# possoj/Spacecraft-Pose-Estimation-Framework

Measured on AMD Instinct MI355X. Metric: images/sec at 512×512 batch 64, 1/2/4/8 MI355X; pose err vs fp32 ref, higher is better.
Workload: dtype fp16mx; 1 GPU; C3: full net + decode, 512x512, batch 64 per GPU, fp16mx schedule; global_batch=64, image_size=512, parallelism=frame-parallel x1 (RCCL weight bcast), inflight_batches=3, frame_buffers=6

## Files before the change

spacecraft-pose-estimation-framework_amd/csrc/api_core.cpp:

```cpp
#include <string.h>

#include <algorithm>

#include "spef_ctx.hpp"

static thread_local std::string g_err;

int fail(int code, const std::string& msg) {
  g_err = msg;
  return code;
}
namespace spef {
int report_error(int code, const std::string& msg) { return fail(code, msg); }
}

int num_cus() {
  static int cus[32] = {};
  int dev = 0;
  if (hipGetDevice(&dev) != hipSuccess) dev = 0;
  dev &= 31;
  if (!cus[dev] && hipDeviceGetAttribute(&cus[dev], hipDeviceAttributeMultiprocessorCount, dev) != hipSuccess)
    cus[dev] = 256;
  return cus[dev];
}
// ... 35 lines not shown
  return SPEF_OK;
}

void free_workspace(spef_ctx* c) {
  for (void*& b : c->buf) {
    if (b) hipFree(b);
    b = nullptr;
  }
  if (c->pooled) hipFree(c->pooled);
  c->pooled = nullptr;
  if (c->kpfeat) hipFree(c->kpfeat);
  c->kpfeat = nullptr;
  if (c->kppart) hipFree(c->kppart);
  c->kppart = nullptr;
  c->ws_B = c->ws_H = c->ws_W = 0;
  c->buf_bytes = 0;
}

struct OptionDesc {
  int option;
  int spef_ctx::*field;
  bool flag;
  int lo, hi;
  const char* msg;
};
static const OptionDesc kOptions[] = {
    {SPEF_OPT_FUSE_BLOCKS, &spef_ctx::fuse, true, 0, 0, nullptr},
    {SPEF_OPT_IRB_VARIANT, &spef_ctx::irb_variant, false, 0, 0, nullptr},
    {SPEF_OPT_TEST_FAIL_BCAST, &spef_ctx::test_fail_bcast, false, 0, 3, "SPEF_OPT_TEST_FAIL_BCAST: 0..3"},
    {SPEF_OPT_PW_GEMM, &spef_ctx::gemm, true, 0, 0, nullptr},
    {SPEF_OPT_Q8_ROLESPLIT, &spef_ctx::q8_rolesplit, false, 0, 1, "SPEF_OPT_Q8_ROLESPLIT: 0 or 1"},
    {SPEF_OPT_MX_KERNELS, &spef_ctx::mx_kernels, true, 0, 0, nullptr},
    {SPEF_OPT_TRIM, &spef_ctx::trim, false, 0, 3, "SPEF_OPT_TRIM: bits 0-1"},
    {SPEF_OPT_WAVESPEC, &spef_ctx::wavespec, false, 0, 2, "SPEF_OPT_WAVESPEC: 0, 1 or 2"},
};

extern "C" {

int spef_abi_version(void) { return SPEF_ABI_VERSION; }

const char* spef_last_error(void) { return g_err.c_str(); }

int spef_init(int device, spef_ctx** out) {
  if (!out) return fail(SPEF_ERR_ARG, "out is null");
  int n = 0;
  HIP_TRY(hipGetDeviceCount(&n));
  if (device < 0 || device >= n) return fail(SPEF_ERR_ARG, "device index out of range");
  hipDeviceProp_t prop;
  HIP_TRY(hipGetDeviceProperties(&prop, device));
  if (strncmp(prop.gcnArchName, "gfx950", 6) != 0)
    return fail(SPEF_ERR_ARG, std::string("SPEF kernels are built for gfx950 only, device is ") + prop.gcnArchName);
  spef_ctx* c = new spef_ctx();
  c->device = device;
  *out = c;
  return SPEF_OK;
}

int spef_destroy(spef_ctx* c) {
  if (!c) return SPEF_OK;
  Dev d(c->device);
  free_workspace(c);
  if (c->d_data) hipFree(c->d_data);
  if (c->d_ori_bins) hipFree(c->d_ori_bins);
  if (c->d_pos_grid) hipFree(c->d_pos_grid);
  if (c->kp3d) hipFree(c->kp3d);
  if (c->kp_model) hipFree(c->kp_model);
// ... 119 lines not shown
```

spacecraft-pose-estimation-framework_amd/csrc/api_schedule.cpp:

```cpp
#include <math.h>

#include <initializer_list>

#include "spef_ctx.hpp"

namespace {

struct Act {
  void* p;
  int h, w, ch;
  bool f16;
};

inline void advance(Act& a, void* y, int h, int w, uint32_t ch, bool f16 = false) { a = Act{y, h, w, (int)ch, f16}; }

void* free_buf(const spef_ctx* c, std::initializer_list<const void*> busy) {
  for (void* b : c->buf) {
    bool used = false;
    for (const void* u : busy) used |= (u == b);
    if (!used) return b;
  }
  return nullptr;
}

// ... 139 lines not shown
int irb_step_x2(const Run& r, const OpDesc& op, const Block& g, Act& a) {
  spef_ctx* c = r.c;
  hipStream_t s = r.s;
  const int B = r.B, h = a.h, w = a.w, OH = g.OH, OW = g.OW;
  void* x = a.p;
  const bool cur16 = a.f16;
  void* y = free_buf(c, {x});
  const double hp = (op.hidden + 31) & ~31u;
  const bool o16 = r.out16(op);
  const int io = (cur16 ? 1 : 0) | (o16 ? 2 : 0);
  float* scratch = (float*)free_buf(c, {x, y});
  const X2Block blk{g.cin, g.hid, g.cout, g.stride, g.expand, g.res};
  const int cus = num_cus();
  const X2Plan plan = x2_irb_plan(blk, B, OH, OW, scratch != nullptr, io, cus);
  if (!plan.known) return fail(SPEF_ERR_ARG, "fp16x2 schedule: unsupported inverted-residual geometry");
  const double ib = cur16 ? 2 : 4, ob = o16 ? 2 : 4;
  const double bytes = (double)g.M * op.cin * ib + (double)g.M2 * op.cout * ob +
                       (g.expand ? hp * ((op.cin + 31) & ~31u) * 4 : 0) + hp * 48 +
                       ((op.cout + 15) & ~15u) * (hp * 4 + 4);
  char key[96];
  const bool mxk = r.mx && c->mx_kernels &&
                   mx_irb_supported(g.cin, g.hid, g.cout, g.stride, g.expand, g.res, cur16, o16);
  const bool mxlean = (c->trim & 2) != 0;
  const char* kn = mxk ? (mxlean && !mx_irb_lean_fits(g.cin, g.cout, o16, h, w, OH, OW) ? "mx_irb_kernel_wide"
                                                                                       : "mx_irb_kernel")
                       : plan.kernel_name();
  snprintf(key, sizeof(key), "%s<%u,%u,%u,s%u>", kn ? kn : "x2_irb_kernel", op.cin, op.hidden, op.cout, op.stride);
  const Wts wt = weights(c, op);
  HIP_TRY(prof_launch(c, s, key, bytes, irb_flops(op, g), [&] {
    if (mxk)
      return launch_mx_irb(g.cin, g.hid, g.cout, g.stride, g.res, cur16, o16, x, wt.w0, wt.b0, (const float*)wt.w1,
                           wt.b1, wt.w2, wt.b2, y, B, h, w, OH, OW, s, mxlean);
    return launch_x2_irb(blk, plan, {x, wt.w0, wt.b0, (const float*)wt.w1, wt.b1, wt.w2, wt.b2, y, B, h, w, OH, OW,
                                     scratch, io, cus}, s);
  }));
  advance(a, y, OH, OW, op.cout, o16);
  return SPEF_OK;
}

bool fused16_applies(const Run& r, const Block& g, const Act& a) {
  return !r.f32 && r.c->fuse && (int64_t)a.h * a.w >= r.c->fuse_min_hw &&
         irb_supported(g.cin, g.hid, g.cout, g.stride, g.expand, g.res);
}

int irb_step_fused16(const Run& r, const OpDesc& op, const Block& g, Act& a) {
  spef_ctx* c = r.c;
  hipStream_t s = r.s;
  const int B = r.B, h = a.h, w = a.w, dt = r.dt, OH = g.OH, OW = g.OW;
  void* x = a.p;
  void* y = free_buf(c, {x});
  const double bytes = (double)g.M * op.cin * 2 + (double)g.M2 * op.cout * 2 +
                       (g.expand ? pw_bytes(0, op.cin, op.hidden, false) : 0) + 40.0 * op.hidden +
                       pw_bytes(0, op.hidden, op.cout, false);
  const bool pipe3 = c->wavespec >= 2 && irp_supported(g.cin, g.hid, g.cout, g.stride, g.expand, g.res);
  const bool wspec = !pipe3 && c->wavespec && irw_supported(g.cin, g.hid, g.cout, g.stride, g.expand, g.res);
  char key[96];
  snprintf(key, sizeof(key), "%s<%u,%u,%u,s%u>", pipe3 ? "irp_kernel" : wspec ? "irw_kernel" : "irb_kernel",
           op.cin, op.hidden, op.cout, op.stride);
  const Wts wt = weights(c, op);
  HIP_TRY(prof_launch(c, s, key, bytes, irb_flops(op, g), [&] {
    if (pipe3)
      return launch_irp(c->irb_variant, dt, g.cin, g.hid, g.cout, g.stride, g.res, x, wt.w0, wt.b0, wt.w1, wt.b1, wt.w2,
                        wt.b2, y, B, h, w, OH, OW, s);
    if (wspec)
      return launch_irw(c->irb_variant, dt, g.cin, g.hid, g.cout, g.stride, g.res, x, wt.w0, wt.b0, wt.w1, wt.b1, wt.w2,
                        wt.b2, y, B, h, w, OH, OW, s);
    return launch_irb(c->irb_variant, dt, g.cin, g.hid, g.cout, g.stride, g.expand, g.res, x, wt.w0, wt.b0, wt.w1,
// ... 437 lines not shown
```

spacecraft-pose-estimation-framework_amd/csrc/k_x2_irw.hip:

```cpp
#include "spef_kernels.hpp"
#include "x2_common.hpp"

namespace spef {

#ifndef SPEF_X2_GLDS
#define SPEF_X2_GLDS 1
#endif
#ifndef SPEF_X2_GLDS_S2
#define SPEF_X2_GLDS_S2 1
#endif
template <int CIN, int HID, int COUT, int S, int TH, int TW, int WCO, bool PST, int P = 1>
struct X2wGeom {
  static constexpr int NE = 4, ND = 4, NW = NE + ND;
  static constexpr int IH = (TH - 1) * S + 3, IW = (TW - 1) * S + 3;
  static constexpr int PIN = IH * IW, PIN16 = (PIN + 15) / 16, PINP = PIN16 * 16;
  static constexpr int CINP = (CIN + 31) / 32 * 32, KS = CINP / 32;
  static constexpr int WES = CINP + 16;
  static constexpr int WPS = 48;
  using SL = X2Slab<S, PINP>;
  static constexpr int NCH = (HID + 31) / 32, HIDP = NCH * 32;
  static constexpr int NCL = NCH / P;
  static constexpr int NCT = (COUT + 15) / 16, NPC = NCT * 16;
  static constexpr int POUT16 = TH * TW / 16;
  static constexpr int WP = ND / WCO, QPW = POUT16 / WP, NCTW = NCT / WCO;
  static constexpr int EPT = (PIN16 + NE - 1) / NE;
  static constexpr int SLAB_B = SL::FLOATS * 4;
  static constexpr int SE_B = 2 * 32 * WES * 2 + 32 * 4;
  static constexpr int SD_B = (9 * 32 + 32) * 4;
  static constexpr int SP_B = PST ? 2 * NPC * WPS * 2 : 0;
  static constexpr bool GL = SPEF_X2_GLDS && COUT == 160 && (S == 1 || SPEF_X2_GLDS_S2);
  static constexpr int SE_BQ = (SE_B + 1023) / 1024 * 1024, SD_BQ = (SD_B + 1023) / 1024 * 1024;
  static constexpr int SP_BQ = (SP_B + 1023) / 1024 * 1024, DP_BQ = SD_BQ + SP_BQ;
  static constexpr int NIE = SE_BQ / 1024, NID = DP_BQ / 1024;
  static constexpr int IEW = (NIE + NE - 1) / NE, IDW = (NID + ND - 1) / ND;
  static constexpr int SE_STR = GL ? SE_BQ : SE_B, SD_STR = GL ? DP_BQ : SD_B, SP_STR = GL ? DP_BQ : SP_B;
  static constexpr int OFF_SE = 2 * SLAB_B;
  static constexpr int OFF_SD = GL ? OFF_SE + 2 * SE_BQ : OFF_SE + 2 * SE_B;
  static constexpr int OFF_SP = GL ? OFF_SD + SD_BQ : OFF_SD + 2 * SD_B;
  static constexpr int OFF_TR = GL ? OFF_SD + 2 * DP_BQ : OFF_SP + 2 * SP_B;
  static constexpr int OFF_ST = OFF_TR + 16 * 24 * 4;
  static constexpr int LDS_BYTES = OFF_ST + (SPEF_X2_STAMP ? 8 * 4 * 64 : 0);
  static constexpr int NPE = 2 * 32 * (CINP / 8) + 8, NPD = 9 * 8 + 8, NPP = PST ? 2 * NPC * 4 : 0;
  static constexpr int NPIECE = (NPE + NPD + NPP + NE * 64 - 1) / (NE * 64);
  static_assert(CIN % 8 == 0 && COUT % 4 == 0 && HID % 8 == 0, "channel counts");
  static_assert(TH * TW % 16 == 0 && POUT16 % WP == 0 && ND % WCO == 0 && NCT % WCO == 0, "tile split");
  static_assert(EPT <= 32 && NCH % P == 0 && NCL >= 2, "validity mask / hidden parts / pipeline depth");
  static_assert(SE_B % 16 == 0 && SD_B % 16 == 0 && SP_B % 16 == 0 && SLAB_B % 16 == 0, "16-B aligned stages");
  static_assert(LDS_BYTES <= 163840, "LDS budget");
};

#ifndef SPEF_X2_DWB
#define SPEF_X2_DWB 2
#endif
#ifndef SPEF_X2_ROWS
#define SPEF_X2_ROWS 1
#endif
#ifndef SPEF_X2_DWB2_CIN
#define SPEF_X2_DWB2_CIN 96
#endif
template <int CIN, int HID, int COUT, int S, int TH, int TW, bool RES, int WCO, bool PST, int P = 1, bool PT = false>
__global__ __launch_bounds__(8 * 64) __attribute__((amdgpu_waves_per_eu(2, 2))) void x2_irw_kernel(
    const float* __restrict__ X, const _Float16* __restrict__ We, const float* __restrict__ be,
    const float* __restrict__ Wd, const float* __restrict__ bd, const _Float16* __restrict__ Wp,
    const float* __restrict__ bp, float* __restrict__ Y, int H, int W, int OH, int OW, int tiles_x, int tiles_y,
    uint32_t nwg, size_t pstride, uint32_t ntile) {
  using G = X2wGeom<CIN, HID, COUT, S, TH, TW, WCO, PST, P>;
  using SL = typename G::SL;
  static_assert(!PT || (P == 1 && G::NCL % 2 == 0), "persistent tiles: one hidden part, even chunk count");
  extern __shared__ __attribute__((aligned(16))) char smem[];
  const int tid = threadIdx.x, wave = tid >> 6, lane = tid & 63;
  const int r16 = lane & 15, kg = lane >> 4;
  uint32_t L = xcd_remap(blockIdx.x, nwg);
  const bool stamp_wg = SPEF_X2_STAMP && L == 0;
  auto stamp = [&](int c, int slot) {
    if constexpr (SPEF_X2_STAMP) {
      if (stamp_wg && lane == 0 && c < 64)
        reinterpret_cast<uint32_t*>(smem + G::OFF_ST)[c * 8 + slot] = (uint32_t)__builtin_amdgcn_s_memtime();
    }
  };
  const uint32_t L0 = L;
  const int nt = PT ? (int)((ntile - L0 + nwg - 1) / nwg) : 1;
  const int GT = nt * G::NCL;
  const int part = (int)(L % (uint32_t)P);
  L /= (uint32_t)P;
  const int cb = part * G::NCL;
  auto tile_of = [&](uint32_t Lt, int& b_, int& oy0_, int& ox0_) {
    const int tx_ = (int)(Lt % (uint32_t)tiles_x);
    Lt /= (uint32_t)tiles_x;
    b_ = (int)(Lt / (uint32_t)tiles_y);
    oy0_ = (int)(Lt % (uint32_t)tiles_y) * TH;
    ox0_ = tx_ * TW;
  };
// ... 492 lines not shown
        if (c == G::NCL - SPEF_X2_RES_AHEAD || c == G::NCL - 1) {
          int b_, oy_, ox_;
          tile_of(L0 + (uint32_t)(g / G::NCL) * nwg, b_, oy_, ox_);
          if (c == G::NCL - SPEF_X2_RES_AHEAD) {
            fetch_res(b_, oy_, ox_);
          } else {
            float4 bn[G::NCTW];
#pragma unroll
            for (int t = 0; t < G::NCTW; ++t)
              bn[t] = *reinterpret_cast<const float4*>(bp + (wc * G::NCTW + t) * 16 + 4 * kg);
            epilogue(b_, oy_, ox_);
#pragma unroll
            for (int t = 0; t < G::NCTW; ++t)
#pragma unroll
              for (int q = 0; q < G::QPW; ++q) acc[q][t] = f32x4{bn[t].x, bn[t].y, bn[t].z, bn[t].w};
          }
        }
      }
      if (wr == 0) stamp(g, 6);
      __syncthreads();
    }
    if constexpr (!PT) epilogue(b, oy0, ox0);
    if (wr == 0) stamp(0, 7);
  }
  if constexpr (SPEF_X2_STAMP) {
    __syncthreads();
    if (stamp_wg && tid < 8 * 64) {
      const int n = 8 * (GT < 64 ? GT : 64);
      if (tid < n) reinterpret_cast<uint32_t*>(Y)[tid] = reinterpret_cast<const uint32_t*>(smem + G::OFF_ST)[tid];
    }
  }
}

template <int P, bool RES>
__global__ __launch_bounds__(256) void x2_split_reduce_kernel(const float* __restrict__ parts, size_t pstride,
                                                              const float* __restrict__ bias,
                                                              const float* __restrict__ X, float* __restrict__ Y,
                                                              size_t n4, int cout4) {
  const size_t i = (size_t)blockIdx.x * 256 + threadIdx.x;
  if (i >= n4) return;
  float4 v = reinterpret_cast<const float4*>(parts)[i];
#pragma unroll
  for (int p = 1; p < P; ++p) {
    const float4 u = reinterpret_cast<const float4*>(parts + p * pstride)[i];
    v.x += u.x; v.y += u.y; v.z += u.z; v.w += u.w;
  }
  const float4 bb = reinterpret_cast<const float4*>(bias)[i % (size_t)cout4];
  v.x += bb.x; v.y += bb.y; v.z += bb.z; v.w += bb.w;
  if constexpr (RES) {
    const float4 r = reinterpret_cast<const float4*>(X)[i];
    v.x += r.x; v.y += r.y; v.z += r.z; v.w += r.w;
  }
  reinterpret_cast<float4*>(Y)[i] = v;
}
template <int CIN, int HID, int COUT, int S, bool EXPAND, bool RES, int TH, int TW, int NW, int WCO, int KIND, int P>
static hipError_t x2_split_go(X2Row<CIN, HID, COUT, S, EXPAND, RES, TH, TW, NW, WCO, KIND, P>, const X2Args& a,
                              hipStream_t s) {
  static_assert(EXPAND && NW == 8, "role-split blocks expand, 4 + 4 waves");
  constexpr bool PT = KIND == 3 && P == 1;
  using G = X2wGeom<CIN, HID, COUT, S, TH, TW, WCO, KIND != 2, P>;
  TileGrid g;
  hipError_t e = tile_grid(g, a.OH, a.OW, TH, TW, a.B, P);
  if (e != hipSuccess) return e;
  auto k = x2_irw_kernel<CIN, HID, COUT, S, TH, TW, RES, WCO, KIND != 2, P, PT>;
  static DevOnce attr_set;
  if ((e = lds_attr_once(attr_set, k, G::LDS_BYTES)) != hipSuccess) return e;
  const size_t pstride = (size_t)a.B * a.OH * a.OW * COUT;
  if (P > 1 && !a.scratch) return hipErrorInvalidValue;
  const uint32_t grid = PT ? x2_persistent_grid(g.nwg, a.num_cu) : g.nwg;
  k<<<grid, G::NW * 64, G::LDS_BYTES, s>>>((const float*)a.x, (const _Float16*)a.we, a.be, a.wd, a.bd,
                                           (const _Float16*)a.wp, a.bp, P > 1 ? a.scratch : (float*)a.y, a.H, a.W,
                                           a.OH, a.OW, g.tiles_x, g.tiles_y, grid, pstride, g.nwg);
  if constexpr (P > 1) {
    const size_t n4 = pstride / 4;
    x2_split_reduce_kernel<P, RES><<<(unsigned)((n4 + 255) / 256), 256, 0, s>>>(a.scratch, pstride, a.bp,
                                                                                 (const float*)a.x, (float*)a.y, n4,
                                                                                 COUT / 4);
  }
  return hipGetLastError();
}

hipError_t launch_x2_split(const X2Block& b, const X2Plan& p, const X2Args& a, hipStream_t s) {
  return x2_visit_row<1, 3>(b, p, hipErrorNotSupported, [&](auto row) { return x2_split_go(row, a, s); });
}

}
```

spacecraft-pose-estimation-framework_amd/csrc/spef_ctx.hpp:

```cpp
#pragma once
#include "../../include/spef.h"

#include <hip/hip_runtime.h>

#include <array>
#include <string>
#include <vector>

#include "spef_blob.hpp"
#include "spef_kernels.hpp"
#include "spef_tuning.hpp"

using namespace spef;

#define SPEF_INTERNAL __attribute__((visibility("hidden")))

static const int kKpSplits = 60;

SPEF_INTERNAL int fail(int code, const std::string& msg);

#define HIP_TRY(expr)                                                                                  \
  do {                                                                                                 \
    hipError_t e_ = (expr);                                                                            \
    if (e_ != hipSuccess) return fail(SPEF_ERR_HIP, std::string(#expr) + ": " + hipGetErrorString(e_)); \
// ... 1 lines not shown

struct spef_ctx {
  int device = 0;
  BlobHeader hdr{};
  std::vector<OpDesc> ops;
  uint8_t* d_data = nullptr;
  size_t data_bytes = 0;
  bool loaded = false;
  int ws_B = 0, ws_H = 0, ws_W = 0;
  size_t buf_bytes = 0;
  void* buf[4] = {nullptr, nullptr, nullptr, nullptr};
  float* pooled = nullptr;
  float* kpfeat = nullptr;
  float* kppart = nullptr;
  float* kp3d = nullptr;
  double* kp_model = nullptr;
  int kp_n = 0;
  double camK[9] = {0};
  float cam_nu = 0.f, cam_nv = 0.f;
  EpnpDist kp_dist = {0, 0, 0, 0, 0, 0};
  double* d_ori_bins = nullptr;
  int n_ori_bins = 0;
  double* d_pos_grid = nullptr;
  int n_pos_bins = 0;
  int fuse = 1;
  int64_t fuse_min_hw = 0;
  int gemm = 1;
  int irb_variant = -1;
  int wavespec = 2;
  int q8_rolesplit = 0;
  int test_fail_bcast = 0;
  int mx_kernels = 1;
  int trim = 3;
  std::vector<double> q8_sw, q8_bias;
  std::vector<int32_t> q8_wsum;
  double q8_sl = 0.0;
  int32_t* q8_fc_init = nullptr;
  float* q8_fc_sc = nullptr;
  int q8_fc_hw = 0, q8_fc_tb = 0;
  float q8_s_img = 0.f;
  int q8_last_bits = 8, q8_pool_bits = 8, q8_fc_bias_bits = 8;
  int pre_key[4] = {0, 0, 0, 0};
  int* pre_bh = nullptr;
  int* pre_bv = nullptr;
  int pre_ksh = 0, pre_ksv = 0, pre_y0 = 0, pre_ht = 0;
  uint8_t* pre_tmp = nullptr;
  size_t pre_tmp_bytes = 0;
  std::vector<std::array<int64_t, 3>> q8_res;
  bool profiling = false;
  struct Rec {
    std::string key;
    hipEvent_t a, b;
    double bytes, flops;
  };
  std::vector<Rec> recs;
  std::vector<hipEvent_t> pool;
  size_t pool_next = 0;
};

struct spef_observer {
  int device = 0;
  int n_blocks = 0, n_taps = 0;
  std::vector<std::array<uint32_t, 7>> geom;
  uint64_t* state = nullptr;
  uint64_t* tap(int t) const { return state + (size_t)t * (OBS_COUNTERS + OBS_BINS); }
};
// ... 68 lines not shown
```

spacecraft-pose-estimation-framework_amd/csrc/spef_kernels.hpp:

```cpp
#pragma once
#include <hip/hip_runtime.h>
#include <stddef.h>
#include <stdint.h>

#include <string>

#include "x2_plan.hpp"

namespace spef {

int report_error(int code, const std::string& msg);

enum Dtype : int {
  DT_F16 = 1, DT_BF16 = 2, DT_I8 = 3, DT_F32 = 4,
  DT_X2 = 5,
  DT_MX = 6
};
enum Epi : int { EPI_NONE = 0, EPI_RELU = 1, EPI_RES = 2, EPI_RELU_F32 = 3  };
enum InLayout : int { IN_U8_NHWC = 0, IN_F32_NCHW = 1 };

hipError_t launch_stem(int dtype, int in_layout, const void* in, const float* w, const float* bias, void* y,
                       int B, int H, int W, int OH, int OW, hipStream_t s);

hipError_t launch_pw(int dtype, int epi, const void* x, const void* wt, const float* bias, const void* r,
// ... 20 lines not shown
int irb_dw_mode(int dtype, int hid, bool expand, int stride);
hipError_t launch_irb(int variant, int dtype, int cin, int hid, int cout, int stride, bool expand, bool res, const void* x,
                      const void* we, const float* be, const void* wd, const float* bd, const void* wp,
                      const float* bp, void* y, int B, int H, int W, int OH, int OW, hipStream_t s);

bool irp_supported(int cin, int hid, int cout, int stride, bool expand, bool res);
hipError_t launch_irp(int variant, int dtype, int cin, int hid, int cout, int stride, bool res, const void* x, const void* we,
                      const float* be, const void* wd, const float* bd, const void* wp, const float* bp, void* y, int B,
                      int H, int W, int OH, int OW, hipStream_t s);
bool irw_supported(int cin, int hid, int cout, int stride, bool expand, bool res);
hipError_t launch_irw(int variant, int dtype, int cin, int hid, int cout, int stride, bool res, const void* x, const void* we,
                      const float* be, const void* wd, const float* bd, const void* wp, const float* bp, void* y,
                      int B, int H, int W, int OH, int OW, hipStream_t s);

hipError_t launch_front(int dtype, const void* x, const void* wsp, const float* bs, const void* wd, const float* bd,
                        const void* wp, const float* bp, void* y, int B, int H, int W, int OH, int OW, hipStream_t s);

hipError_t launch_gemm_f32(int epi, const void* x, const void* wt, const float* bias, const void* r, void* y,
                           int64_t M, int K, int N, hipStream_t s);
const char* gemm_f32_key(int N);
bool x2_irb_supported(int cin, int hid, int cout, int stride, bool expand, bool res);
const char* x2_irb_kernel_name(int cin, int hid, int cout, int stride, bool expand, bool res, int B, int OH, int OW,
                               bool scratch, int io, int num_cu);
struct X2Args {
  const void* x;
  const void* we;
  const float *be, *wd, *bd;
  const void* wp;
  const float* bp;
  void* y;
  int B, H, W, OH, OW;
  float* scratch;
  int io, num_cu;
};
hipError_t launch_x2_irb(const X2Block& b, const X2Plan& p, const X2Args& a, hipStream_t s);
hipError_t launch_x2_slab(const X2Block& b, const X2Plan& p, const X2Args& a, hipStream_t s);
hipError_t launch_x2_split(const X2Block& b, const X2Plan& p, const X2Args& a, hipStream_t s);
hipError_t launch_x2_stage3(const X2Block& b, const X2Plan& p, const X2Args& a, hipStream_t s);
bool mx_irb_supported(int cin, int hid, int cout, int stride, bool expand, bool res, bool in16, bool out16);
hipError_t launch_mx_irb(int cin, int hid, int cout, int stride, bool res, bool in16, bool out16, const void* x,
                         const void* we,
                         const float* be, const float* wd, const float* bd, const void* wp, const float* bp, void* y,
                         int B, int H, int W, int OH, int OW, hipStream_t s, bool lean = true);
bool mx_irb_lean_fits(int cin, int cout, bool out16, int H, int W, int OH, int OW);
hipError_t launch_mx_front(const void* x, const void* wsp, const float* bs, const float* wd, const float* bd,
                           const void* wp, const float* bp, void* y, int B, int H, int W, int OH, int OW,
                           hipStream_t s);
hipError_t launch_x2_front(const void* x, const void* wsx, const float* bs, const float* wd, const float* bd,
                           const void* wp, const float* bp, void* y, int B, int H, int W, int OH, int OW, hipStream_t s,
                           bool out16 = false);
hipError_t launch_x2_pw_relu(const void* x, const void* wt, const float* bias, float* y, int64_t M, int K, int N,
                             hipStream_t s, bool wide = true);
bool x2_pw_pool_supported(int HW, int N);
hipError_t launch_x2_pw_pool(const void* x, const void* wt, const float* bias, float* part, float* pooled, int B,
                             int HW, int K, int N, hipStream_t s, bool wide = true);
hipError_t launch_mean_hw(const float* x, float* pooled, int B, int HW, int C, hipStream_t s);

hipError_t launch_fc_splitk(const float* x, const float* w, const float* bias, float* out, int n, int B, int K,
                            int splits, float* part, hipStream_t s);

struct EpnpDist {
  double k1, k2, p1, p2, k3;
  int on;
};
hipError_t launch_epnp(const float* raw, int B, int n, const float* kp3d, const double* model, const double* K,
                       float nu, float nv, const EpnpDist& dist, int apply_sigmoid, float* kp_out, float* quat,
// ... 132 lines not shown
```

spacecraft-pose-estimation-framework_amd/csrc/spef_tuning.hpp:

```cpp
#pragma once

enum spef_tuning_option {
  SPEF_OPT_FUSE_MIN_HW = 2,
  SPEF_OPT_PW_GEMM = 3,
  SPEF_OPT_IRB_VARIANT = 4,
  SPEF_OPT_TEST_FAIL_BCAST = 5,
  SPEF_OPT_MX_KERNELS = 8,
  SPEF_OPT_TRIM = 9
};
```

spacecraft-pose-estimation-framework_amd/spef_amd/_lib.py:

```python
from __future__ import annotations

import ctypes as C
import os

from . import _build

OK, ERR_ARG, ERR_HIP, ERR_BLOB, ERR_STATE, ERR_NUMERIC, ERR_COMM = range(7)
IN_U8_NHWC, IN_F32_NCHW = 0, 1
REGRESSION, CLASSIFICATION, KEYPOINTS = 0, 1, 2
ABI_VERSION = 4
COMM_ID_BYTES = 128
METRIC_IDS = {'l2': 0, 'kl': 1, 'js': 2, 'hellinger': 3, 'tv': 4, 'wasserstein': 5}
OPT_FUSE_BLOCKS, OPT_WAVESPEC, OPT_Q8_ROLESPLIT = 1, 6, 7
OPT_FUSE_MIN_HW, OPT_PW_GEMM, OPT_IRB_VARIANT, OPT_TEST_FAIL_BCAST = 2, 3, 4, 5
OPT_MX_KERNELS = 8
OPT_TRIM = 9
OPT_TRIM_DEFAULT = 3

_vp, _i, _sz = C.c_void_p, C.c_int, C.c_size_t
_ip = C.POINTER(C.c_int)
SIGNATURES = {
    'spef_abi_version': (_i, []),
    'spef_last_error': (C.c_char_p, []),
    'spef_init': (_i, [_i, C.POINTER(_vp)]),
    'spef_destroy': (_i, [_vp]),
    'spef_load_weights': (_i, [_vp, _vp, _sz]),
    'spef_load_weights_device': (_i, [_vp, _vp, _sz]),
    'spef_model_info': (_i, [_vp, _ip, _ip, _ip, _ip, _ip]),
    'spef_reserve': (_i, [_vp, _i, _i, _i]),
    'spef_preprocess': (_i, [_vp, _vp, _i, _i, _i, _vp, _i, _i, _vp]),
    'spef_forward': (_i, [_vp, _vp, _i, _i, _i, _i, _vp, _vp, _vp]),
    'spef_backbone': (_i, [_vp, _vp, _i, _i, _i, _i, _vp, _vp]),
    'spef_probe': (_i, [_vp, _vp, _i, _i, _i, _i, _i, _vp, _ip, _ip, _ip, _vp]),
    'spef_set_decode_tables': (_i, [_vp, _vp, _i, _vp, _i]),
    'spef_decode': (_i, [_vp, _i, _i, _vp, _i, _vp, _i, _i, _vp, _vp, _vp, _vp, _vp, _vp]),
    'spef_decode_cov': (_i, [_vp, _i, _i, _vp, _i, _vp, _i, _vp, _vp, _i, _vp, _vp, _vp, _vp, _vp]),
    'spef_video_create': (_i, [_vp, _i, _i, C.c_float, C.c_float, C.c_float, C.c_float, C.POINTER(_vp)]),
    'spef_video_reset': (_i, [_vp, _i, _vp]),
    'spef_video_set_state': (_i, [_vp, _i, _vp, _vp, _vp, _vp, _vp]),
    'spef_video_step': (_i, [_vp, _vp, _vp, _vp, _i, _i, _vp, _vp, _vp, _vp, _vp, _vp, _vp, _vp, _vp]),
    'spef_video_destroy': (_i, [_vp]),
    'spef_score_create': (_i, [_vp, _i, _i, _i, C.POINTER(_vp)]),
    'spef_score_reset': (_i, [_vp, _i, _vp]),
    'spef_score_step': (_i, [_vp, _i, _vp, _vp, _vp, _vp, _vp, _i, _i, _vp, _vp]),
    'spef_score_finalize': (_i, [_vp, _vp, _vp]),
    'spef_score_log': (_i, [_vp, _i, _i, _i, _i, _vp, _vp, _vp]),
    'spef_score_destroy': (_i, [_vp]),
    'spef_track_create': (_i, [_vp, _i, _vp, C.POINTER(_vp)]),
    'spef_track_reset': (_i, [_vp, _i, _vp]),
    'spef_track_get_state': (_i, [_vp, _i, _i, _vp, _vp]),
# ... 89 lines not shown
```

Baseline: 61390 images/sec.

## Add warp-specialized staged x2 IRB kernel with async global-to-LDS weight pipeline

```diff
diff --git a/spacecraft-pose-estimation-framework_amd/csrc/api_core.cpp b/spacecraft-pose-estimation-framework_amd/csrc/api_core.cpp
--- a/spacecraft-pose-estimation-framework_amd/csrc/api_core.cpp
+++ b/spacecraft-pose-estimation-framework_amd/csrc/api_core.cpp
@@ -91,6 +91,7 @@
     {SPEF_OPT_Q8_ROLESPLIT, &spef_ctx::q8_rolesplit, false, 0, 1, "SPEF_OPT_Q8_ROLESPLIT: 0 or 1"},
     {SPEF_OPT_MX_KERNELS, &spef_ctx::mx_kernels, true, 0, 0, nullptr},
     {SPEF_OPT_TRIM, &spef_ctx::trim, false, 0, 3, "SPEF_OPT_TRIM: bits 0-1"},
+    {SPEF_OPT_X2_STAGE, &spef_ctx::x2_stage, false, 0, 1, "SPEF_OPT_X2_STAGE: 0 or 1"},
     {SPEF_OPT_WAVESPEC, &spef_ctx::wavespec, false, 0, 2, "SPEF_OPT_WAVESPEC: 0, 1 or 2"},
 };
 
diff --git a/spacecraft-pose-estimation-framework_amd/csrc/api_schedule.cpp b/spacecraft-pose-estimation-framework_amd/csrc/api_schedule.cpp
--- a/spacecraft-pose-estimation-framework_amd/csrc/api_schedule.cpp
+++ b/spacecraft-pose-estimation-framework_amd/csrc/api_schedule.cpp
@@ -195,7 +195,7 @@
       return launch_mx_irb(g.cin, g.hid, g.cout, g.stride, g.res, cur16, o16, x, wt.w0, wt.b0, (const float*)wt.w1,
                            wt.b1, wt.w2, wt.b2, y, B, h, w, OH, OW, s, mxlean);
     return launch_x2_irb(blk, plan, {x, wt.w0, wt.b0, (const float*)wt.w1, wt.b1, wt.w2, wt.b2, y, B, h, w, OH, OW,
-                                     scratch, io, cus}, s);
+                                     scratch, io, cus, c->x2_stage}, s);
   }));
   advance(a, y, OH, OW, op.cout, o16);
   return SPEF_OK;
diff --git a/spacecraft-pose-estimation-framework_amd/csrc/k_x2_irw.hip b/spacecraft-pose-estimation-framework_amd/csrc/k_x2_irw.hip
--- a/spacecraft-pose-estimation-framework_amd/csrc/k_x2_irw.hip
+++ b/spacecraft-pose-estimation-framework_amd/csrc/k_x2_irw.hip
@@ -8,6 +8,9 @@
 #endif
 #ifndef SPEF_X2_GLDS_S2
 #define SPEF_X2_GLDS_S2 1
+#endif
+#ifndef SPEF_X2_DPE_WIDE
+#define SPEF_X2_DPE_WIDE 0
 #endif
 template <int CIN, int HID, int COUT, int S, int TH, int TW, int WCO, bool PST, int P = 1>
 struct X2wGeom {
@@ -47,7 +50,82 @@
   static_assert(EPT <= 32 && NCH % P == 0 && NCL >= 2, "validity mask / hidden parts / pipeline depth");
   static_assert(SE_B % 16 == 0 && SD_B % 16 == 0 && SP_B % 16 == 0 && SLAB_B % 16 == 0, "16-B aligned stages");
   static_assert(LDS_BYTES <= 163840, "LDS budget");
+  static constexpr int SLF = SL::FLOATS + 16 * 24;
+  static constexpr int DPE = COUT == 64 ? NID : SPEF_X2_DPE_WIDE < NID ? SPEF_X2_DPE_WIDE : NID;
+  static constexpr int ST_LDS = 2 * SLF * 4 + 2 * SE_BQ + 2 * DP_BQ + (SPEF_X2_STAMP ? 8 * 4 * 64 : 0);
 };
+
+template <class G>
+__device__ __forceinline__ const char* x2w_stage_src(bool estage, int off, const _Float16* We, const float* be,
+                                                     const float* Wd, const float* bd, const _Float16* Wp) {
+  if (estage) {
+    constexpr int EW_B = 2 * 32 * G::WES * 2, ROW_B = G::WES * 2;
+    if (off < EW_B) {
+      const int pl = off / (32 * ROW_B), rem = off - pl * (32 * ROW_B), rr = rem / ROW_B;
+      const int col = (rem - rr * ROW_B) / 16;
+      return reinterpret_cast<const char*>(We + (size_t)pl * G::HIDP * G::CINP + (size_t)rr * G::CINP +
+                                           (col < G::CINP / 8 ? 8 * col : 0));
+    }
+    const int g = (off - EW_B) / 16;
+    return reinterpret_cast<const char*>(be + (g < 8 ? 4 * g : 0));
+  }
+  if (off < 1152) return reinterpret_cast<const char*>(Wd + (size_t)(off / 128) * G::HIDP + 4 * ((off % 128) / 16));
+  if (off < G::SD_BQ) {
+    const int g = (off - 1152) / 16;
+    return reinterpret_cast<const char*>(bd + (g < 8 ? 4 * g : 0));
+  }
+  const int o2 = off - G::SD_BQ;
+  constexpr int ROW_B = G::WPS * 2;
+  const int pl = o2 / (G::NPC * ROW_B), rem = o2 - pl * (G::NPC * ROW_B), rr = rem / ROW_B;
+  const int q = (rem - rr * ROW_B) / 16;
+  const bool ok = o2 < G::SP_B;
+  return reinterpret_cast<const char*>(Wp + (ok ? (size_t)pl * G::NPC * G::HIDP + (size_t)rr * G::HIDP : 0) +
+                                       (ok && q < 4 ? 8 * q : 0));
+}
+template <class G>
+__device__ __forceinline__ int x2w_stage_stride(bool estage, int off) {
+  return estage ? (off < 2 * 32 * G::WES * 2 ? 32 * G::CINP * 2 : 128) : off < G::SD_BQ ? 128 : 64;
+}
+
+template <class G>
+__device__ __forceinline__ void x2w_expand(const char* S0, float* Sl, const f16x8 (&bxh)[G::EPT][G::KS],
+                                           const f16x8 (&bxl)[G::EPT][G::KS], uint32_t pvmask,
+                                           const int (&soff)[G::EPT], int r16, int kg) {
+  const float* eb = reinterpret_cast<const float*>(S0 + 2 * 32 * G::WES * 2);
+  f32x4 acc[G::EPT][2];
+#pragma unroll
+  for (int h = 0; h < 2; ++h) {
+    const float4 bb = *reinterpret_cast<const float4*>(eb + 16 * h + 4 * kg);
+#pragma unroll
+    for (int j = 0; j < G::EPT; ++j) acc[j][h] = f32x4{bb.x, bb.y, bb.z, bb.w};
+  }
+  const _Float16* Ws = reinterpret_cast<const _Float16*>(S0);
+#pragma unroll
+  for (int ks = 0; ks < G::KS; ++ks) {
+    f16x8 ah[2], al[2];
+#pragma unroll
+    for (int h = 0; h < 2; ++h) {
+      ah[h] = *reinterpret_cast<const f16x8*>(Ws + (16 * h + r16) * G::WES + 32 * ks + 8 * kg);
+      al[h] = *reinterpret_cast<const f16x8*>(Ws + (32 + 16 * h + r16) * G::WES + 32 * ks + 8 * kg);
+    }
+#pragma unroll
+    for (int j = 0; j < G::EPT; ++j) {
+#pragma unroll
+      for (int h = 0; h < 2; ++h) acc[j][h] = mfma_x2(ah[h], al[h], bxh[j][ks], bxl[j][ks], acc[j][h]);
+    }
+  }
+#pragma unroll
+  for (int j = 0; j < G::EPT; ++j) {
+    const bool pv = (pvmask >> j) & 1u;
+#pragma unroll
+    for (int h = 0; h < 2; ++h) {
+      float4 v = make_float4(fmaxf(acc[j][h][0], 0.f), fmaxf(acc[j][h][1], 0.f), fmaxf(acc[j][h][2], 0.f),
+                             fmaxf(acc[j][h][3], 0.f));
+      if (!pv) v = make_float4(0.f, 0.f, 0.f, 0.f);
+      *reinterpret_cast<float4*>(Sl + soff[j] + 8 * h) = v;
+    }
+  }
+}
 
 #ifndef SPEF_X2_DWB
 #define SPEF_X2_DWB 2
@@ -58,6 +136,91 @@
 #ifndef SPEF_X2_DWB2_CIN
 #define SPEF_X2_DWB2_CIN 96
 #endif
+template <class G, int CIN, int S, int TW, class Mid>
+__device__ __forceinline__ void x2w_dwproj(const float* Sl, const float* D, const _Float16* Ps,
+                                           const int (&pbase)[G::QPW], f32x4 (&acc)[G::QPW][G::NCTW], int wc, int r16,
+                                           int kg, Mid mid) {
+  using SL = typename G::SL;
+  f32x2 a[G::QPW][4];
+  {
+    const float4 d0 = *reinterpret_cast<const float4*>(D + 288 + 8 * kg);
+    const float4 d1 = *reinterpret_cast<const float4*>(D + 288 + 8 * kg + 4);
+#pragma unroll
+    for (int q = 0; q < G::QPW; ++q) {
+      a[q][0] = f32x2{d0.x, d0.y}; a[q][1] = f32x2{d0.z, d0.w};
+      a[q][2] = f32x2{d1.x, d1.y}; a[q][3] = f32x2{d1.z, d1.w};
+    }
+  }
+  constexpr int DWB = (SPEF_X2_DWB == 2 && G::QPW > 1 && CIN > SPEF_X2_DWB2_CIN) ? 1 : SPEF_X2_DWB;
+  if constexpr (DWB > 0) {
+    constexpr bool ROWS = SPEF_X2_ROWS && S == 1 && TW == 16 && G::QPW > 1;
+    constexpr int NR = ROWS ? G::QPW + 2 : 3 * G::QPW;
+    float4 wv[DWB][3][2], sr[DWB][NR][2];
+    auto col = [&](int kx, int bf) {
+#pragma unroll
+      for (int ky = 0; ky < 3; ++ky) {
+        const float* wt = D + (ky * 3 + kx) * 32 + 8 * kg;
+        wv[bf][ky][0] = *reinterpret_cast<const float4*>(wt);
+        wv[bf][ky][1] = *reinterpret_cast<const float4*>(wt + 4);
+      }
+#pragma unroll
+      for (int r = 0; r < NR; ++r) {
+        const int p = ROWS ? pbase[0] + r * G::IW + kx : pbase[r % G::QPW] + (r / G::QPW) * G::IW + kx;
+        sr[bf][r][0] = *reinterpret_cast<const float4*>(Sl + SL::at(p, 2 * kg));
+        sr[bf][r][1] = *reinterpret_cast<const float4*>(Sl + SL::at(p, 2 * kg + 1));
+      }
+    };
+    col(0, 0);
+#pragma unroll
+    for (int kx = 0; kx < 3; ++kx) {
+      const int bf = DWB == 2 ? (kx & 1) : 0;
+      if (DWB == 2 && kx < 2) col(kx + 1, bf ^ 1);
+      __builtin_amdgcn_sched_barrier(0);
+#pragma unroll
+      for (int ky = 0; ky < 3; ++ky) {
+        const float4 w0 = wv[bf][ky][0], w1 = wv[bf][ky][1];
+        const f32x2 w4[4] = {f32x2{w0.x, w0.y}, f32x2{w0.z, w0.w}, f32x2{w1.x, w1.y}, f32x2{w1.z, w1.w}};
+#pragma unroll
+        for (int q = 0; q < G::QPW; ++q) {
+          const int r = ROWS ? q + ky : ky * G::QPW + q;
+          dw_tap8(a[q], sr[bf][r][0], sr[bf][r][1], w4);
+        }
+      }
+      if (DWB == 1 && kx < 2) {
+        __builtin_amdgcn_sched_barrier(0);
+        col(kx + 1, 0);
+      }
+    }
+  } else {
+#pragma unroll
+    for (int kx = 0; kx < 3; ++kx)
+#pragma unroll
+      for (int ky = 0; ky < 3; ++ky) {
+        const float* wt = D + (ky * 3 + kx) * 32 + 8 * kg;
+        const float4 w0 = *reinterpret_cast<const float4*>(wt), w1 = *reinterpret_cast<const float4*>(wt + 4);
+        const f32x2 w4[4] = {f32x2{w0.x, w0.y}, f32x2{w0.z, w0.w}, f32x2{w1.x, w1.y}, f32x2{w1.z, w1.w}};
+#pragma unroll
+        for (int q = 0; q < G::QPW; ++q) {
+          const int p = pbase[q] + ky * G::IW + kx;
+          dw_tap8(a[q], *reinterpret_cast<const float4*>(Sl + SL::at(p, 2 * kg)),
+                  *reinterpret_cast<const float4*>(Sl + SL::at(p, 2 * kg + 1)), w4);
+        }
+      }
+  }
+  f16x8 bh[G::QPW], bl[G::QPW];
+#pragma unroll
+  for (int q = 0; q < G::QPW; ++q) relu_split8(a[q], bh[q], bl[q]);
+  mid();
+#pragma unroll
+  for (int t = 0; t < G::NCTW; ++t) {
+    const int row = (wc * G::NCTW + t) * 16 + r16;
+    const f16x8 ph = *reinterpret_cast<const f16x8*>(Ps + row * G::WPS + 8 * kg);
+    const f16x8 pl = *reinterpret_cast<const f16x8*>(Ps + (G::NPC + row) * G::WPS + 8 * kg);
+#pragma unroll
+    for (int q = 0; q < G::QPW; ++q) acc[q][t] = mfma_x2(ph, pl, bh[q], bl[q], acc[q][t]);
+  }
+}
+
 template <int CIN, int HID, int COUT, int S, int TH, int TW, bool RES, int WCO, bool PST, int P = 1, bool PT = false>
 __global__ __launch_bounds__(8 * 64) __attribute__((amdgpu_waves_per_eu(2, 2))) void x2_irw_kernel(
     const float* __restrict__ X, const _Float16* __restrict__ We, const float* __restrict__ be,
@@ -616,6 +779,281 @@
   }
 }
 
+template <class G, bool EW>
+struct X2wPieces {
+  static constexpr int N = EW ? G::NIE + G::DPE : G::NID - G::DPE, NJ = (N + 3) / 4;
+  static_assert(G::DPE >= 0 && G::DPE <= G::NID, "pieces moved to the expand waves");
+  static_assert(2 * 32 * G::WES * 2 % 1024 == 0 && G::SD_BQ % 1024 == 0, "a piece has one chunk stride");
+  const char* src[NJ ? NJ : 1];
+  int kstr[NJ ? NJ : 1], poff[NJ ? NJ : 1], wr;
+  __device__ __forceinline__ X2wPieces(int wr_, int lane, const _Float16* We, const float* be, const float* Wd,
+                                       const float* bd, const _Float16* Wp)
+      : wr(wr_) {
+#pragma unroll
+    for (int j = 0; j < NJ; ++j) {
+      const int i = wr + 4 * j;
+      const bool es = EW && i < G::NIE;
+      poff[j] = (es ? i : EW ? G::NID - G::DPE + (i - G::NIE) : i) * 1024;
+      src[j] = x2w_stage_src<G>(es, poff[j] + lane * 16, We, be, Wd, bd, Wp);
+      kstr[j] = x2w_stage_stride<G>(es, poff[j]);
+    }
+  }
+  template <bool E, bool D>
+  __device__ __forceinline__ void issue(int ke, char* ebuf, int kd, char* dbuf) const {
+#pragma unroll
+    for (int j = 0; j < NJ; ++j) {
+      const int i = wr + 4 * j;
+      const bool es = EW && i < G::NIE;
+      if (i < N && (es ? E : D))
+        __builtin_amdgcn_global_load_lds((const void*)(src[j] + (size_t)(es ? ke : kd) * kstr[j]),
+                                         (__attribute__((address_space(3))) void*)((es ? ebuf : dbuf) + poff[j]), 16, 0,
+                                         0);
+    }
+  }
+};
+
+template <int CIN, int HID, int COUT, int S, int TH, int TW, bool RES, int WCO>
+__global__ __launch_bounds__(8 * 64) __attribute__((amdgpu_waves_per_eu(2, 2))) void x2_irw_st_kernel(
+    const float* __restrict__ X, const _Float16* __restrict__ We, const float* __restrict__ be,
+    const float* __restrict__ Wd, const float* __restrict__ bd, const _Float16* __restrict__ Wp,
+    const float* __restrict__ bp, float* __restrict__ Y, int H, int W, int OH, int OW, int tiles_x, int tiles_y,
+    uint32_t nwg, uint32_t ntile) {
+  using G = X2wGeom<CIN, HID, COUT, S, TH, TW, WCO, true, 1>;
+  using SL = typename G::SL;
+  static_assert(G::NCL % 2 == 0 && G::ST_LDS <= 163840, "even chunk count (parity of a global chunk) / LDS budget");
+  __shared__ __attribute__((aligned(16))) float Sl0[G::SLF], Sl1[G::SLF];
+  __shared__ __attribute__((aligned(1024))) char Se0[G::SE_BQ], Se1[G::SE_BQ];
+  __shared__ __attribute__((aligned(1024))) char Sd0[G::DP_BQ], Sd1[G::DP_BQ];
+  __shared__ __attribute__((aligned(16))) float Sb[G::NPC];
+  __shared__ uint32_t Stamps[SPEF_X2_STAMP ? 8 * 64 : 1];
+  using I0 = std::integral_constant<int, 0>;
+  using I1 = std::integral_constant<int, 1>;
+  auto slab = [&](auto p) -> float* { if constexpr (decltype(p)::value) return Sl1; else return Sl0; };
+  auto se = [&](auto p) -> char* { if constexpr (decltype(p)::value) return Se1; else return Se0; };
+  auto sd = [&](auto p) -> char* { if constexpr (decltype(p)::value) return Sd1; else return Sd0; };
+
+  const int tid = threadIdx.x, wave = __builtin_amdgcn_readfirstlane(tid >> 6), lane = tid & 63;
+  const int r16 = lane & 15, kg = lane >> 4;
+  const uint32_t L0 = xcd_remap(blockIdx.x, nwg);
+  const int nt = (int)((ntile - L0 + nwg - 1) / nwg);
+  const int GT = nt * G::NCL;
+  auto tile_of = [&](int t, int& b_, int& oy0_, int& ox0_) {
+    uint32_t Lt = L0 + (uint32_t)t * nwg;
+    const int tx_ = (int)(Lt % (uint32_t)tiles_x);
+    Lt /= (uint32_t)tiles_x;
+    b_ = (int)(Lt / (uint32_t)tiles_y);
+    oy0_ = (int)(Lt % (uint32_t)tiles_y) * TH;
+    ox0_ = tx_ * TW;
+  };
+  const bool stamp_wg = SPEF_X2_STAMP && L0 == 0;
+  auto stamp = [&](int c, int slot) {
+    if constexpr (SPEF_X2_STAMP) {
+      if (stamp_wg && lane == 0 && c < 64) Stamps[c * 8 + slot] = (uint32_t)__builtin_amdgcn_s_memtime();
+    }
+  };
+  const bool ewave = wave < G::NE;
+  static_assert(G::NE == 4 && G::ND == 4, "4 + 4 waves");
+  const int wr = wave & 3;
+  if (wave == 0) stamp(0, 3);
+  if (wave == G::NE) stamp(1, 7);
+
+  if (ewave) {
+    const int e = wr;
+    const X2wPieces<G, true> pieces(wr, lane, We, be, Wd, bd, Wp);
+    pieces.template issue<true, true>(0, Se0, 0, Sd0);
+    pieces.template issue<true, false>(1, Se1, 0, Sd1);
+    f16x8 bxh[G::EPT][G::KS], bxl[G::EPT][G::KS];
+    uint32_t pvmask = 0;
+    int soff[G::EPT];
+    auto pix = [&](int j, int iy0_, int ix0_, int& iy, int& ix) {
+      const int p = (e + G::NE * j) * 16 + r16;
+      if (p >= G::PIN) return false;
+      const int py = p / G::IW, px = p - py * G::IW;
+      iy = iy0_ + py;
+      ix = ix0_ + px;
+      return iy >= 0 && iy < H && ix >= 0 && ix < W;
+    };
+    auto load_raw = [&](int t) {
+      int b_, oy_, ox_;
+      tile_of(t, b_, oy_, ox_);
+      const float* Xb = X + (size_t)b_ * H * W * CIN;
+#pragma unroll
+      for (int j = 0; j < G::EPT; ++j) {
+        int iy = 0, ix = 0;
+        const bool ok = pix(j, oy_ * S - 1, ox_ * S - 1, iy, ix);
+#pragma unroll
+        for (int ks = 0; ks < G::KS; ++ks) {
+          const int ch = 32 * ks + 8 * kg;
+          float4 r0 = make_float4(0.f, 0.f, 0.f, 0.f), r1 = r0;
+          if (ok && ch < CIN) {
+            const float* src = Xb + ((size_t)iy * W + ix) * CIN + ch;
+            r0 = *reinterpret_cast<const float4*>(src);
+            r1 = *reinterpret_cast<const float4*>(src + 4);
+          }
+          bxh[j][ks] = __builtin_bit_cast(f16x8, r0);
+          bxl[j][ks] = __builtin_bit_cast(f16x8, r1);
+        }
+      }
+    };
+    auto split_mask = [&](int t) {
+      int b_, oy_, ox_;
+      tile_of(t, b_, oy_, ox_);
+      pvmask = 0;
+#pragma unroll
+      for (int j = 0; j < G::EPT; ++j) {
+        const int p = (e + G::NE * j) * 16 + r16;
+        int iy, ix;
+        if (pix(j, oy_ * S - 1, ox_ * S - 1, iy, ix)) pvmask |= 1u << j;
+        soff[j] = p < G::PINP ? SL::at(p, kg) : SL::FLOATS + r16 * 24 + 4 * kg;
+#pragma unroll
+        for (int ks = 0; ks < G::KS; ++ks) {
+          const float4 a = __builtin_bit_cast(float4, bxh[j][ks]), c = __builtin_bit_cast(float4, bxl[j][ks]);
+          const float v8[8] = {a.x, a.y, a.z, a.w, c.x, c.y, c.z, c.w};
+          split8(v8, bxh[j][ks], bxl[j][ks]);
+        }
+      }
+    };
+    load_raw(0);
+    split_mask(0);
+    if (wave == 0) stamp(1, 3);
+    __builtin_amdgcn_s_waitcnt(0x0F70);
+    __syncthreads();
+    x2w_expand<G>(Se0, Sl0, bxh, bxl, pvmask, soff, r16, kg);
+    __syncthreads();
+    auto iter = [&](auto par, int g) {
+      using Q = std::integral_constant<int, decltype(par)::value ^ 1>;
+      if (wave == 0) stamp(g, 0);
+      const bool more = g + 1 < GT;
+      const int cn = (g + 1) % G::NCL, tn = (g + 1) / G::NCL;
+      __builtin_amdgcn_s_waitcnt(0x0F70);
+      if (more && cn == 0) split_mask(tn);
+      pieces.template issue<true, true>((g + 2) % G::NCL, se(par), cn, sd(Q{}));
+      if (wave == 0) stamp(g, 2);
+      if (more) x2w_expand<G>(se(Q{}), slab(Q{}), bxh, bxl, pvmask, soff, r16, kg);
+      __builtin_amdgcn_s_waitcnt(0x0F70);
+      if (more && cn == G::NCL - 1 && tn + 1 < nt) load_raw(tn + 1);
+      if (wave == 0) stamp(g, 1);
+      lds_barrier();
+    };
+#pragma unroll 1
+    for (int g = 0; g < GT; g += 2) {
+      iter(I0{}, g);
+      iter(I1{}, g + 1);
+    }
+  } else {
+    const int d = wr;
+    const X2wPieces<G, false> pieces(wr, lane, We, be, Wd, bd, Wp);
+    pieces.template issue<false, true>(0, Se0, 0, Sd0);
+    const int wp = d % G::WP, wc = d / G::WP;
+    const int co0 = wc * G::NCTW * 16 + 4 * kg;
+    auto co_here = [&] {
+      int c_ = co0;
+      asm volatile("" : "+v"(c_));
+      return c_;
+    };
+    f32x4 acc[G::QPW][G::NCTW];
+#pragma unroll
+    for (int t = 0; t < G::NCTW; ++t) {
+      const float4 bb = *reinterpret_cast<const float4*>(bp + co0 + 16 * t);
+      *reinterpret_cast<float4*>(Sb + co0 + 16 * t) = bb;
+#pragma unroll
+      for (int q = 0; q < G::QPW; ++q) acc[q][t] = f32x4{bb.x, bb.y, bb.z, bb.w};
+    }
+    int pbase[G::QPW];
+#pragma unroll
+    for (int q = 0; q < G::QPW; ++q) {
+      const int o = (wp * G::QPW + q) * 16 + r16;
+      const int oy = o / TW, ox = o - (o / TW) * TW;
+      pbase[q] = oy * S * G::IW + ox * S;
+    }
+    static_assert(COUT % 16 == 0 && (!RES || CIN == COUT), "whole output-channel tiles; a residual block keeps its width");
+    constexpr int NRES = RES ? G::QPW * G::NCTW : 1;
+    float4 rres[NRES];
+    auto out_pix = [&](int q, int b_, int oy0_, int ox0_, size_t& pix_) {
+      const int o = (wp * G::QPW + q) * 16 + r16;
+      const int oy = o / TW, ox = o - (o / TW) * TW;
+      const int gy = oy0_ + oy, gx = ox0_ + ox;
+      pix_ = ((size_t)b_ * OH + gy) * OW + gx;
+      return gy < OH && gx < OW;
+    };
+    auto fetch_res = [&](int b_, int oy0_, int ox0_) {
+      if constexpr (RES) {
+#pragma unroll
+        for (int q = 0; q < G::QPW; ++q) {
+          size_t pix_;
+          const bool in = out_pix(q, b_, oy0_, ox0_, pix_);
+          const float* xp = X + pix_ * CIN + co_here();
+#pragma unroll
+          for (int t = 0; t < G::NCTW; ++t)
+            rres[q * G::NCTW + t] = in && (wc * G::NCTW + t) * 16 < COUT ? *reinterpret_cast<const float4*>(xp + 16 * t)
+                                                                       : make_float4(0.f, 0.f, 0.f, 0.f);
+        }
+      }
+    };
+    auto epilogue = [&](int b_, int oy0_, int ox0_) {
+#pragma unroll
+      for (int q = 0; q < G::QPW; ++q) {
+        size_t pix;
+        if (!out_pix(q, b_, oy0_, ox0_, pix)) continue;
+        float* yp = Y + pix * COUT + co_here();
+#pragma unroll
+        for (int t = 0; t < G::NCTW; ++t) {
+          if ((wc * G::NCTW + t) * 16 >= COUT) continue;
+          f32x4 v = acc[q][t];
+          if constexpr (RES) {
+            const float4 r = rres[q * G::NCTW + t];
+            v[0] += r.x; v[1] += r.y; v[2] += r.z; v[3] += r.w;
+          }
+          *reinterpret_cast<float4*>(yp + 16 * t) = make_float4(v[0], v[1], v[2], v[3]);
+        }
+      }
+    };
+    __builtin_amdgcn_s_waitcnt(0x0F70);
+    __syncthreads();
+    __syncthreads();
+    auto iter = [&](auto par, int g) {
+      using Q = std::integral_constant<int, decltype(par)::value ^ 1>;
+      const int c = g % G::NCL;
+      if (wr == 0) stamp(g, 4);
+      pieces.template issue<false, true>(0, se(par), (g + 1) % G::NCL, sd(Q{}));
+      x2w_dwproj<G, CIN, S, TW>(slab(par), reinterpret_cast<const float*>(sd(par)),
+                                reinterpret_cast<const _Float16*>(sd(par) + G::SD_BQ), pbase, acc, wc, r16, kg,
+                                [&] { if (wr == 0) stamp(g, 5); });
+      __builtin_amdgcn_s_waitcnt(0x0F70);
+      if (c == G::NCL - SPEF_X2_RES_AHEAD || c == G::NCL - 1) {
+        int b_, oy_, ox_;
+        tile_of(g / G::NCL, b_, oy_, ox_);
+        if (c == G::NCL - SPEF_X2_RES_AHEAD) {
+          fetch_res(b_, oy_, ox_);
+        } else {
+          epilogue(b_, oy_, ox_);
+#pragma unroll
+          for (int t = 0; t < G::NCTW; ++t) {
+            const float4 bn = *reinterpret_cast<const float4*>(Sb + co0 + 16 * t);
+#pragma unroll
+            for (int q = 0; q < G::QPW; ++q) acc[q][t] = f32x4{bn.x, bn.y, bn.z, bn.w};
+          }
+        }
+      }
+      if (wr == 0) stamp(g, 6);
+      lds_barrier();
+    };
+#pragma unroll 1
+    for (int g = 0; g < GT; g += 2) {
+      iter(I0{}, g);
+      iter(I1{}, g + 1);
+    }
+    if (wr == 0) stamp(0, 7);
+  }
+  if constexpr (SPEF_X2_STAMP) {
+    __syncthreads();
+    if (stamp_wg) {
+      const int n = 8 * (GT < 64 ? GT : 64);
+      if (tid < n) reinterpret_cast<uint32_t*>(Y)[tid] = Stamps[tid];
+    }
+  }
+}
+
 template <int P, bool RES>
 __global__ __launch_bounds__(256) void x2_split_reduce_kernel(const float* __restrict__ parts, size_t pstride,
                                                               const float* __restrict__ bias,
@@ -646,6 +1084,15 @@
   TileGrid g;
   hipError_t e = tile_grid(g, a.OH, a.OW, TH, TW, a.B, P);
   if (e != hipSuccess) return e;
+  if constexpr (PT) {
+    if (a.stage) {
+      const uint32_t grid = x2_persistent_grid(g.nwg, a.num_cu);
+      x2_irw_st_kernel<CIN, HID, COUT, S, TH, TW, RES, WCO><<<grid, G::NW * 64, 0, s>>>(
+          (const float*)a.x, (const _Float16*)a.we, a.be, a.wd, a.bd, (const _Float16*)a.wp, a.bp, (float*)a.y, a.H,
+          a.W, a.OH, a.OW, g.tiles_x, g.tiles_y, grid, g.nwg);
+      return hipGetLastError();
+    }
+  }
   auto k = x2_irw_kernel<CIN, HID, COUT, S, TH, TW, RES, WCO, KIND != 2, P, PT>;
   static DevOnce attr_set;
   if ((e = lds_attr_once(attr_set, k, G::LDS_BYTES)) != hipSuccess) return e;
diff --git a/spacecraft-pose-estimation-framework_amd/csrc/spef_ctx.hpp b/spacecraft-pose-estimation-framework_amd/csrc/spef_ctx.hpp
--- a/spacecraft-pose-estimation-framework_amd/csrc/spef_ctx.hpp
+++ b/spacecraft-pose-estimation-framework_amd/csrc/spef_ctx.hpp
@@ -57,6 +57,7 @@
   int test_fail_bcast = 0;
   int mx_kernels = 1;
   int trim = 3;
+  int x2_stage = 1;
   std::vector<double> q8_sw, q8_bias;
   std::vector<int32_t> q8_wsum;
   double q8_sl = 0.0;
diff --git a/spacecraft-pose-estimation-framework_amd/csrc/spef_kernels.hpp b/spacecraft-pose-estimation-framework_amd/csrc/spef_kernels.hpp
--- a/spacecraft-pose-estimation-framework_amd/csrc/spef_kernels.hpp
+++ b/spacecraft-pose-estimation-framework_amd/csrc/spef_kernels.hpp
@@ -76,6 +76,7 @@
   int B, H, W, OH, OW;
   float* scratch;
   int io, num_cu;
+  int stage = 1;
 };
 hipError_t launch_x2_irb(const X2Block& b, const X2Plan& p, const X2Args& a, hipStream_t s);
 hipError_t launch_x2_slab(const X2Block& b, const X2Plan& p, const X2Args& a, hipStream_t s);
diff --git a/spacecraft-pose-estimation-framework_amd/csrc/spef_tuning.hpp b/spacecraft-pose-estimation-framework_amd/csrc/spef_tuning.hpp
--- a/spacecraft-pose-estimation-framework_amd/csrc/spef_tuning.hpp
+++ b/spacecraft-pose-estimation-framework_amd/csrc/spef_tuning.hpp
@@ -6,5 +6,6 @@
   SPEF_OPT_IRB_VARIANT = 4,
   SPEF_OPT_TEST_FAIL_BCAST = 5,
   SPEF_OPT_MX_KERNELS = 8,
-  SPEF_OPT_TRIM = 9
+  SPEF_OPT_TRIM = 9,
+  SPEF_OPT_X2_STAGE = 10
 };
diff --git a/spacecraft-pose-estimation-framework_amd/spef_amd/_lib.py b/spacecraft-pose-estimation-framework_amd/spef_amd/_lib.py
--- a/spacecraft-pose-estimation-framework_amd/spef_amd/_lib.py
+++ b/spacecraft-pose-estimation-framework_amd/spef_amd/_lib.py
@@ -16,6 +16,8 @@
 OPT_MX_KERNELS = 8
 OPT_TRIM = 9
 OPT_TRIM_DEFAULT = 3
+OPT_X2_STAGE = 10
+OPT_X2_STAGE_DEFAULT = 1
 
 _vp, _i, _sz = C.c_void_p, C.c_int, C.c_size_t
 _ip = C.POINTER(C.c_int)
```

Measured after the change: 62700 images/sec (median of 6 runs). 1.02x the previous value.
